# jnvance/DMRG.x

Measured on AMD Instinct MI355X. Metric: superblock MatMults/sec inside the ground-state eigensolve (Lanczos step = 1 MatMult + reorthogonalisation), higher is better.
Workload: dtype f64

## Files before the change

### dmrg.x_amd/csrc/ggemm.hip

```cpp
#include "ggemm.h"
#include <algorithm>
#include <cstdlib>
#include <map>
#include <mutex>
#include <utility>

namespace dmrgx {

typedef double d4 __attribute__((ext_vector_type(4)));

#ifdef DMRGX_TILE_TRACE
#define GG_TRACE_PARAM , unsigned long long* __restrict__ trace
#define GG_STAMP(I) { if (trace && threadIdx.x == 0) trace[(size_t)t * 8 + (I)] = __builtin_amdgcn_s_memrealtime(); }
#define GG_STAMP_ID() { if (trace && threadIdx.x == 0) { unsigned hw, xcc; asm volatile("s_getreg_b32 %0, hwreg(HW_REG_HW_ID)" : "=s"(hw)); asm volatile("s_getreg_b32 %0, hwreg(HW_REG_XCC_ID)" : "=s"(xcc)); trace[(size_t)t * 8 + 7] = ((unsigned long long)xcc << 32) | hw; } }
#define GG_TRACE_FWD , trace
#define GG_CLK0() unsigned long long clk0_ = __builtin_amdgcn_s_memtime();
#define GG_CLK1() { if (trace && threadIdx.x == 0) trace[(size_t)t * 8 + 6] = __builtin_amdgcn_s_memtime() - clk0_; }
#else
#define GG_TRACE_PARAM
#define GG_TRACE_FWD
#define GG_STAMP(I)
#define GG_STAMP_ID()
#define GG_CLK0()
#define GG_CLK1()
#endif
typedef const double __attribute__((address_space(1)))* gptr;
typedef double __attribute__((address_space(1)))* gwptr;
typedef const char __attribute__((address_space(1)))* gbptr;

typedef const GTile __attribute__((address_space(4)))* ktile_ptr;
typedef const GGroup __attribute__((address_space(4)))* kgroup_ptr;
typedef const GProd __attribute__((address_space(4)))* kprod_ptr;
__device__ __forceinline__ GTile kload(ktile_ptr p, int i) { GTile r; r.group = p[i].group; r.tm = p[i].tm; r.tn = p[i].tn; r.pad = p[i].pad; return r; }
__device__ __forceinline__ GGroup kload(kgroup_ptr p, int i)
{
    GGroup r;
    r.C = p[i].C; r.ldc = p[i].ldc; r.M = p[i].M; r.N = p[i].N; r.prod_begin = p[i].prod_begin; r.prod_end = p[i].prod_end;
    r.n_axpy = p[i].n_axpy; r.accumulate = p[i].accumulate;
    return r;
}
__device__ __forceinline__ GProd kload(kprod_ptr p, int i)
{
    GProd r;
    r.A = p[i].A; r.B = p[i].B; r.lda = p[i].lda; r.ldb = p[i].ldb; r.K = p[i].K; r.kind = p[i].kind; r.alpha = p[i].alpha;
    return r;
}


template <int TR, int TC, int WR, int WC, bool DEEP>
__device__ __forceinline__ void
ggemm_body(const GTile* __restrict__ tiles_, const GGroup* __restrict__ groups_, const GProd* __restrict__ prods_, int ntiles, int* __restrict__ ctr GG_TRACE_PARAM)
{
    const ktile_ptr tiles = (ktile_ptr)tiles_;
    const kgroup_ptr groups = (kgroup_ptr)groups_;
    const kprod_ptr prods = (kprod_ptr)prods_;
    constexpr int THREADS = 64 * WR * WC;
    constexpr int BM = 16 * TR * WR, BN = 16 * TC * WC, BK = GG_BK;
    constexpr int AS_LD = BK + 2;
    constexpr int BS_LD = BN + 16;
    constexpr int AROWS = THREADS / 16;
    constexpr int NA = BM / AROWS;
    constexpr int BROWS = THREADS / BN;
    constexpr int NB = BK / BROWS;
    constexpr bool RELAYOUT = (TR == 2 && TC == 2 && WR == 2 && WC == 2);
    extern __shared__ double gg_smem[];
    double (*As)[BM * AS_LD] = (double (*)[BM * AS_LD])gg_smem;
    double (*Bs)[BK * BS_LD] = (double (*)[BK * BS_LD])(gg_smem + 2 * BM * AS_LD);

    const int tid = threadIdx.x, wave = __builtin_amdgcn_readfirstlane(tid >> 6);
    int& sh_next = *(int*)(gg_smem + 2 * BM * AS_LD + 2 * BK * BS_LD);
    const int G = gridDim.x;
    const bool dyn = ntiles > G;
    const int xcd = blockIdx.x & 7, qbase = G >> 3;
    int t = blockIdx.x;
    GTile tl = kload(tiles, t);
    if (tl.group < 0) return;
    GGroup g = kload(groups, tl.group);
    const GTile tl_none = GTile{-1, 0, 0, 0};
#define GG_LANES()                                                                            \
    int tp_ = tid;                                                                            \
    asm volatile("" : "+v"(tp_));                                                             \
    const int a_r = tp_ >> 4, a_k = tp_ & 15, b_k = tp_ / BN, b_j = tp_ % BN;                 \
    (void)a_r; (void)a_k; (void)b_k; (void)b_j;
    unsigned st_a, st_b;
    {
        GG_LANES();
        st_a = (unsigned)(size_t)&As[0][a_r * AS_LD + a_k];
        st_b = (unsigned)(size_t)&Bs[0][b_k * BS_LD + b_j];
    }

    int lm0, ln0, lmrem, lnrem;
    double rc_a[NA], rc_b[NB];
    const double *cA = nullptr, *cB = nullptr;
    int clda = 0, cldb = 0, cK = 0;
    int lp = 0, lk = 0, lpend = 0;
    bool lmore = false;
    int kz[2] = {0, 0};
    int npre = 0;
    int vm_after = 0;

#define GG_LOADER_TILE(TL, GR)                                                                \
    {                                                                                         \
        lm0 = (TL).tm * GG_BM; ln0 = (TL).tn * GG_BN;                                         \
        lmrem = min(BM, (GR).M - lm0);                                                        \
        lnrem = min(BN, (GR).N - ln0);                                                        \
    }
#define GG_PRODUCT_SET(PR)                                                                    \
    {                                                                                         \
        cA = (PR).A; cB = (PR).B; clda = (PR).lda; cldb = (PR).ldb; cK = (PR).K;              \
        const int kc_ = min(cK, BK) - 1;                                                      \
        GG_LANES();                                                                           \
        const int bcol = min(b_j, lnrem - 1);                                                 \
        _Pragma("unroll") for (int s = 0; s < NA; ++s) aoff[s] = ((unsigned)min(a_r + AROWS * s, lmrem - 1) * (unsigned)clda + (unsigned)min(a_k, kc_)) * 8u; \
        _Pragma("unroll") for (int s = 0; s < NB; ++s) boff[s] = ((unsigned)min(b_k + BROWS * s, kc_) * (unsigned)cldb + (unsigned)bcol) * 8u; \
    }
#define GG_PRODUCT(P) { const GProd pr_ = kload(prods, P); GG_PRODUCT_SET(pr_); }
#define GG_RA_0_0 "v[96:97]"
#define GG_CA_0_0 "v96", "v97"
#define GG_RA_0_1 "v[98:99]"
#define GG_CA_0_1 "v98", "v99"
#define GG_RA_0_2 "v[100:101]"
#define GG_CA_0_2 "v100", "v101"
#define GG_RA_0_3 "v[102:103]"
#define GG_CA_0_3 "v102", "v103"
#define GG_RB_0_0 "v[104:105]"
#define GG_CB_0_0 "v104", "v105"
#define GG_RB_0_1 "v[106:107]"
#define GG_CB_0_1 "v106", "v107"
#define GG_RB_0_2 "v[108:109]"
#define GG_CB_0_2 "v108", "v109"
#define GG_RB_0_3 "v[110:111]"
#define GG_CB_0_3 "v110", "v111"
#define GG_RA_1_0 "v[112:113]"
#define GG_CA_1_0 "v112", "v113"
#define GG_RA_1_1 "v[114:115]"
#define GG_CA_1_1 "v114", "v115"
#define GG_RA_1_2 "v[116:117]"
#define GG_CA_1_2 "v116", "v117"
#define GG_RA_1_3 "v[118:119]"
#define GG_CA_1_3 "v118", "v119"
#define GG_RB_1_0 "v[120:121]"
#define GG_CB_1_0 "v120", "v121"
#define GG_RB_1_1 "v[122:123]"
#define GG_CB_1_1 "v122", "v123"
#define GG_RB_1_2 "v[124:125]"
#define GG_CB_1_2 "v124", "v125"
#define GG_RB_1_3 "v[126:127]"
#define GG_CB_1_3 "v126", "v127"
#define GG_ZT_0_0 "v_cndmask_b32_e64 v96, v96, 0, %0\n\tv_cndmask_b32_e64 v97, v97, 0, %0"
#define GG_ZT_0_1 "v_cndmask_b32_e64 v98, v98, 0, %0\n\tv_cndmask_b32_e64 v99, v99, 0, %0"
#define GG_ZT_0_2 "v_cndmask_b32_e64 v100, v100, 0, %0\n\tv_cndmask_b32_e64 v101, v101, 0, %0"
#define GG_ZT_0_3 "v_cndmask_b32_e64 v102, v102, 0, %0\n\tv_cndmask_b32_e64 v103, v103, 0, %0"
#define GG_ZT_1_0 "v_cndmask_b32_e64 v112, v112, 0, %0\n\tv_cndmask_b32_e64 v113, v113, 0, %0"
#define GG_ZT_1_1 "v_cndmask_b32_e64 v114, v114, 0, %0\n\tv_cndmask_b32_e64 v115, v115, 0, %0"
#define GG_ZT_1_2 "v_cndmask_b32_e64 v116, v116, 0, %0\n\tv_cndmask_b32_e64 v117, v117, 0, %0"
#define GG_ZT_1_3 "v_cndmask_b32_e64 v118, v118, 0, %0\n\tv_cndmask_b32_e64 v119, v119, 0, %0"
#define GG_LD1(OP, SET, S, OFFV, BASE, BREG) asm volatile("global_load_dwordx2 " GG_R##OP##_##SET##_##S ", %0, %1" : : "v"(OFFV), BREG(BASE) : "memory", GG_C##OP##_##SET##_##S)
#define GG_ST1(OP, SET, S, ADDR, OFFS) asm volatile("ds_write_b64 %0, " GG_R##OP##_##SET##_##S " offset:%1" : : "v"(ADDR), "i"(OFFS) : "memory")
#define GG_Z1(SET, S) asm volatile(GG_ZT_##SET##_##S : : "s"(zm_) : GG_CA_##SET##_##S)
#define GG_LOADER_NEXT()                                                                      \
    {                                                                                         \
        lk += BK;                                                                             \
        if (lk >= cK) { ++lp; lk = 0; if (lp < lpend) GG_PRODUCT(lp); }                       \
        lmore = lp < lpend;                                                                   \
    }
#define GG_LOADER_BASES()                                                                     \
        const int klast_ = cK - 1 - lk;                                                       \
        const int back_ = (klast_ < BK - 1 && cK >= BK) ? BK - 1 - klast_ : 0;                \
        const int kz_ = klast_ < BK - 1 ? (cK >= BK ? back_ : -(klast_ + 1)) : 0;             \
        gbptr A_ = (gbptr)(cA + (size_t)lm0 * clda + (lk - back_));                           \
        gbptr B_ = (gbptr)(cB + (size_t)(lk - back_) * cldb + ln0);
#define GG_GLOAD_D(SET)                                                                       \
    {                                                                                         \
        static_assert(!DEEP || (NA == 4 && NB == 4), "staging register table");               \
        GG_LOADER_BASES();                                                                    \
        kz[SET] = kz_;                                                                        \
        GG_LD1(A, SET, 0, aoff[0], A_, "{s[96:97]}"); GG_LD1(A, SET, 1, aoff[1 % NA], A_, "{s[96:97]}");   \
        GG_LD1(A, SET, 2, aoff[2 % NA], A_, "{s[96:97]}"); GG_LD1(A, SET, 3, aoff[3 % NA], A_, "{s[96:97]}");   \
        GG_LD1(B, SET, 0, boff[0], B_, "{s[98:99]}"); GG_LD1(B, SET, 1, boff[1 % NB], B_, "{s[98:99]}");   \
        GG_LD1(B, SET, 2, boff[2 % NB], B_, "{s[98:99]}"); GG_LD1(B, SET, 3, boff[3 % NB], B_, "{s[98:99]}");   \
        GG_LOADER_NEXT();                                                                     \
    }
#define GG_VMWAIT(N) asm volatile("s_waitcnt vmcnt(%0)" : : "n"(N) : "memory")
#define GG_LSTORE_D(BUF, SET)                                                                 \
    {                                                                                         \
        if (kz[SET] != 0) {                                                                   \
            GG_LANES();                                                                       \
            const unsigned long long zm_ = __builtin_amdgcn_ballot_w64(kz[SET] > 0 ? a_k < kz[SET] : a_k >= -kz[SET]);   \
            GG_Z1(SET, 0); GG_Z1(SET, 1); GG_Z1(SET, 2); GG_Z1(SET, 3);                       \
        }                                                                                     \
        GG_ST1(A, SET, 0, st_a, 8 * ((BUF) * BM * AS_LD + AROWS * 0 * AS_LD)); GG_ST1(A, SET, 1, st_a, 8 * ((BUF) * BM * AS_LD + AROWS * 1 * AS_LD)); \
        GG_ST1(A, SET, 2, st_a, 8 * ((BUF) * BM * AS_LD + AROWS * 2 * AS_LD)); GG_ST1(A, SET, 3, st_a, 8 * ((BUF) * BM * AS_LD + AROWS * 3 * AS_LD)); \
        GG_ST1(B, SET, 0, st_b, 8 * ((BUF) * BK * BS_LD + BROWS * 0 * BS_LD)); GG_ST1(B, SET, 1, st_b, 8 * ((BUF) * BK * BS_LD + BROWS * 1 * BS_LD)); \
        GG_ST1(B, SET, 2, st_b, 8 * ((BUF) * BK * BS_LD + BROWS * 2 * BS_LD)); GG_ST1(B, SET, 3, st_b, 8 * ((BUF) * BK * BS_LD + BROWS * 3 * BS_LD)); \
    }
#define GG_GLOAD_C()                                                                          \
    {                                                                                         \
        GG_LOADER_BASES();                                                                    \
        kz[0] = kz_;                                                                          \
        _Pragma("unroll") for (int s = 0; s < NA; ++s) rc_a[s] = *(gptr)(A_ + aoff[s]);       \
        _Pragma("unroll") for (int s = 0; s < NB; ++s) rc_b[s] = *(gptr)(B_ + boff[s]);       \
        GG_LOADER_NEXT();                                                                     \
    }
#define GG_LSTORE_C(BUF)                                                                      \
    {                                                                                         \
        if (kz[0] != 0) {                                                                     \
            GG_LANES();                                                                       \
            const bool z_ = kz[0] > 0 ? a_k < kz[0] : a_k >= -kz[0];                          \
            _Pragma("unroll") for (int s = 0; s < NA; ++s) rc_a[s] = z_ ? 0.0 : rc_a[s];      \
        }                                                                                     \
        _Pragma("unroll") for (int s = 0; s < NA; ++s)                                        \
            asm volatile("ds_write_b64 %0, %1 offset:%2" : : "v"(st_a), "v"(rc_a[s]), "i"(8 * ((BUF) * BM * AS_LD + AROWS * s * AS_LD)) : "memory"); \
        _Pragma("unroll") for (int s = 0; s < NB; ++s)                                        \
            asm volatile("ds_write_b64 %0, %1 offset:%2" : : "v"(st_b), "v"(rc_b[s]), "i"(8 * ((BUF) * BK * BS_LD + BROWS * s * BS_LD)) : "memory"); \
    }

#define GG_FRAG(SET, BUF, KK)                                                                 \
    {                                                                                         \
        _Pragma("unroll") for (int mi = 0; mi < TR; ++mi)                                     \
            asm volatile("ds_read_b64 %0, %1 offset:%2" : "=v"(fa[SET][mi]) : "v"(lds_a), "i"(8 * ((BUF) * BM * AS_LD + 16 * AS_LD * mi + (KK))) : "memory"); \
        _Pragma("unroll") for (int ni = 0; ni < TC; ++ni)                                     \
            asm volatile("ds_read_b64 %0, %1 offset:%2" : "=v"(fb[SET][ni]) : "v"(lds_b), "i"(8 * ((BUF) * BK * BS_LD + (KK) * BS_LD + 16 * ni)) : "memory"); \
    }
#define GG_FRAG_WAIT(SET)                                                                     \
    {                                                                                         \
        asm volatile("s_waitcnt lgkmcnt(0)" ::: "memory");                                    \
        _Pragma("unroll") for (int mi = 0; mi < TR; ++mi) asm volatile("" : "+v"(fa[SET][mi])); \
        _Pragma("unroll") for (int ni = 0; ni < TC; ++ni) asm volatile("" : "+v"(fb[SET][ni])); \
    }
#define GG_MFMA(SET, GUARD, I0, I1)       \
    {                                                                                         \
        _Pragma("unroll") for (int q = (I0); q < (I1); ++q) {                                 \
            const int mi = q / TC, ni = q % TC;                                               \
            GUARD(acc[mi][ni], fa[SET][mi], fb[SET][ni], q);                                  \
        }                                                                                     \
        __builtin_amdgcn_sched_barrier(0);                                                    \
    }
#define GG_CLAIM()                                                                            \
    asm volatile("s_mov_b64 s[94:95], exec\n\ts_mov_b64 exec, 1\n\tglobal_atomic_add %0, %1, %2, %3 sc0\n\ts_mov_b64 exec, s[94:95]" \
                 : "+v"(claim) : "v"(0u), "v"(1u), "{s[92:93]}"(ctr + xcd) : "memory", "s94", "s95")
#define GG_STEP_D(BUF, OTH, GUARD)                                                            \
    {                                                                                         \
        constexpr int NM = TR * TC;                                                           \
        GG_FRAG_WAIT(0);                                                                      \
        GG_MFMA(0, GUARD, 0, 1);                                                              \
        const bool ld_ = lmore;                                                               \
        __builtin_amdgcn_sched_barrier(0);                                                    \
        GG_MFMA(0, GUARD, 1, 2);                                                              \
        if (ld_) {                                                                            \
            GG_GLOAD_D(BUF);                                                                  \
            if (dyn && !lmore && wave == 0) GG_CLAIM();    \
        }                                                                                     \
        __builtin_amdgcn_sched_barrier(0);                                                    \
        GG_MFMA(0, GUARD, 2, NM - 1);                                                         \
        GG_FRAG(1, BUF, 4);                                                                   \
        GG_MFMA(0, GUARD, NM - 1, NM);                                                        \
        GG_FRAG_WAIT(1);                                                                      \
        GG_MFMA(1, GUARD, 0, NM - 1);                                                         \
        GG_FRAG(0, BUF, 8);                                                                   \
        GG_MFMA(1, GUARD, NM - 1, NM);                                                        \
        GG_FRAG_WAIT(0);                                                                      \
        GG_MFMA(0, GUARD, 0, 1);                                                              \
        if (have1) {                                                                          \
            if (ld_ && lmore) { GG_VMWAIT(NA + NB); } else { GG_VMWAIT(0); }    \
            GG_LSTORE_D(OTH, OTH);                                                            \
        }                                                                                     \
        __builtin_amdgcn_sched_barrier(0);                                                    \
        GG_MFMA(0, GUARD, 1, NM - 1);                                                         \
        GG_FRAG(1, BUF, 12);                                                                  \
        GG_MFMA(0, GUARD, NM - 1, NM);                                                        \
        GG_FRAG_WAIT(1);                                                                      \
        __syncthreads();                                                                      \
        if (have1) GG_FRAG(0, OTH, 0);                                                        \
        __builtin_amdgcn_sched_barrier(0);                                                    \
        GG_MFMA(1, GUARD, 0, NM);                                                             \
        have = have1; have1 = ld_;                                                            \
    }
#define GG_STEP_C(BUF, OTH, GUARD)                                                            \
    {                                                                                         \
        constexpr int NM = TR * TC;                                                           \
        GG_FRAG_WAIT(0);                                                                      \
        GG_MFMA(0, GUARD, 0, 1);                                                              \
        const bool ld_ = lmore;                                                               \
        __builtin_amdgcn_sched_barrier(0);                                                    \
        GG_MFMA(0, GUARD, 1, 2);                                                              \
        if (ld_) {                                                                            \
            GG_GLOAD_C();                                                                     \
            if (dyn && !lmore && wave == 0) GG_CLAIM();                                       \
        }                                                                                     \
        __builtin_amdgcn_sched_barrier(0);                                                    \
        GG_MFMA(0, GUARD, 2, NM - 1);                                                         \
        GG_FRAG(1, BUF, 4);                                                                   \
        GG_MFMA(0, GUARD, NM - 1, NM);                                                        \
        GG_FRAG_WAIT(1);                                                                      \
        GG_MFMA(1, GUARD, 0, NM - 1);                                                         \
        GG_FRAG(0, BUF, 8);                                                                   \
        GG_MFMA(1, GUARD, NM - 1, NM);                                                        \
        GG_FRAG_WAIT(0);                                                                      \
        GG_MFMA(0, GUARD, 0, 1);                                                              \
        if (ld_) GG_LSTORE_C(OTH);                                                            \
        __builtin_amdgcn_sched_barrier(0);                                                    \
        GG_MFMA(0, GUARD, 1, NM - 1);                                                         \
        GG_FRAG(1, BUF, 12);                                                                  \
        GG_MFMA(0, GUARD, NM - 1, NM);                                                        \
        GG_FRAG_WAIT(1);                                                                      \
        __syncthreads();                                                                      \
        if (ld_) GG_FRAG(0, OTH, 0);                                                          \
        __builtin_amdgcn_sched_barrier(0);                                                    \
        GG_MFMA(1, GUARD, 0, NM);                                                             \
        have = ld_;                                                                           \
    }
#define GG_STREAM(GUARD)                                                                      \
    while (have) {                                                                            \
        if (DEEP) { GG_STEP_D(0, 1, GUARD); } else { GG_STEP_C(0, 1, GUARD); }                \
        if (!have) break;                                                                     \
        if (DEEP) { GG_STEP_D(1, 0, GUARD); } else { GG_STEP_C(1, 0, GUARD); }                \
    }

    for (;;) {
        GG_STAMP(0);
        unsigned aoff[NA], boff[NB];
        const int m0 = tl.tm * GG_BM, n0 = tl.tn * GG_BN;
        const int mrem = min(BM, g.M - m0), nrem = min(BN, g.N - n0);
        int wrow = (wave / WC) * 16 * TR, wcol = (wave % WC) * 16 * TC;
        int tr_eff, tc_eff;
        if (RELAYOUT && mrem <= 32) {
            wrow = 0; wcol = 16 * wave;
            tr_eff = (mrem + 15) >> 4; tc_eff = nrem > wcol ? 1 : 0;
        } else if (RELAYOUT && nrem <= 32) {
            wrow = 16 * wave; wcol = 0;
            tr_eff = mrem > wrow ? 1 : 0; tc_eff = (nrem + 15) >> 4;
        } else {
            tr_eff = min(TR, max(0, (mrem - wrow + 15) >> 4)); tc_eff = min(TC, max(0, (nrem - wcol + 15) >> 4));
        }
        unsigned lds_a, lds_b;
        {
            int tf = tid;
            asm volatile("" : "+v"(tf));
            const int l15 = tf & 15, l4 = (tf >> 4) & 3;
            lds_a = (unsigned)(size_t)&As[0][(wrow + l15) * AS_LD + l4];
            lds_b = (unsigned)(size_t)&Bs[0][l4 * BS_LD + wcol + l15];
        }
        double fa[2][TR], fb[2][TC];

        d4 acc[TR][TC];
#pragma unroll
        for (int mi = 0; mi < TR; ++mi)
#pragma unroll
            for (int ni = 0; ni < TC; ++ni) acc[mi][ni] = (d4){0.0, 0.0, 0.0, 0.0};

        const int pend = g.prod_end;
        const int p0 = tl.pad >= 0 ? tl.pad : pend;
        if (npre == 0 && p0 < pend) {
            GG_LOADER_TILE(tl, g);
            lp = p0; lk = 0; lpend = pend;
            GG_PRODUCT(lp);
            GG_STAMP(1);
            vm_after = 0;
            if (DEEP) { GG_GLOAD_D(0); npre = 1; if (lmore) { GG_GLOAD_D(1); npre = 2; vm_after = NA + NB; } }
            else { GG_GLOAD_C(); npre = 1; }
        } else if (lmore) {
            GG_PRODUCT(lp);
        } else {
#pragma unroll
            for (int s = 0; s < NA; ++s) aoff[s] = 0u;
#pragma unroll
            for (int s = 0; s < NB; ++s) boff[s] = 0u;
        }
        bool have = npre >= 1, have1 = npre >= 2;
        (void)have1;
        if (have) {
            if (DEEP) {
                if (vm_after == NA + NB) { GG_VMWAIT(NA + NB); }
                else if (vm_after == NA + NB + TR * TC * 4) { GG_VMWAIT(NA + NB + TR * TC * 4); }
                else if (vm_after == TR * TC * 4) { GG_VMWAIT(TR * TC * 4); }
                else { GG_VMWAIT(0); }
                GG_LSTORE_D(0, 0);
            } else GG_LSTORE_C(0);
        }
        npre = 0;
        unsigned claim = 0xffffffffu;
        if (dyn && have && !lmore && wave == 0) GG_CLAIM();
        __syncthreads();
        GG_STAMP(2);
        GG_CLK0();
        if (have) GG_FRAG(0, 0, 0);
        unsigned gmask = 0;
#pragma unroll
        for (int q = 0; q < TR * TC; ++q) gmask |= ((q / TC) < tr_eff && (q % TC) < tc_eff) ? (1u << q) : 0u;
gmask = __builtin_amdgcn_readfirstlane(gmask);
#define GG_ALL(ACC, FA, FB, Q) ACC = __builtin_amdgcn_mfma_f64_16x16x4f64(FA, FB, ACC, 0, 0, 0)
#define GG_BIT(ACC, FA, FB, Q)                                                                \
        asm volatile("s_bitcmp1_b32 %3, %4\n\ts_cbranch_scc0 1f\n\tv_mfma_f64_16x16x4_f64 %0, %1, %2, %0\n1:" : "+v"(ACC) : "v"(FA), "v"(FB), "s"(gmask), "n"(Q) : "scc")
        if (TR * TC > 6) { GG_STREAM(GG_ALL) }
        else { GG_STREAM(GG_BIT) }
        GG_STAMP(3);
        GG_CLK1();
#pragma unroll
        for (int s = 0; s < NA; ++s) asm volatile("" : "=v"(rc_a[s]));
#pragma unroll
        for (int s = 0; s < NB; ++s) asm volatile("" : "=v"(rc_b[s]));
        int t_n = ntiles;
        if (dyn) {
            asm volatile("s_waitcnt vmcnt(0)" : "+v"(claim) : : "memory");
            if (tid == 0) sh_next = claim != 0xffffffffu ? (int)claim : (int)atomicAdd(&ctr[xcd], 1);
            __syncthreads();
            t_n = xcd + 8 * (__builtin_amdgcn_readfirstlane(sh_next) + qbase);
        }
        const GTile tl_n = t_n < ntiles ? kload(tiles, t_n) : tl_none;
        const bool nx = tl_n.group >= 0;
        GGroup g_n = g;
        GProd pr_n = GProd{nullptr, nullptr, 0, 0, 0, 0, 0.0};
        if (nx) g_n = kload(groups, tl_n.group);
        if (nx && tl_n.pad >= 0) pr_n = kload(prods, tl_n.pad);

        int tq = tid;
        asm volatile("" : "+v"(tq));
        const int el15 = tq & 15, el4 = (tq >> 4) & 3;
        const int erow = wrow + el4, ecol = wcol + el15;
        int q = g.prod_begin;
        const int axpy_end = q + g.n_axpy;
        const bool full_tile = mrem == BM && nrem == BN;
        if (DEEP && full_tile && q < axpy_end) {
#define GG_SREG_0 "v[96:97]"
#define GG_SCLB_0 "v96", "v97"
#define GG_SREG_1 "v[98:99]"
#define GG_SCLB_1 "v98", "v99"
#define GG_SREG_2 "v[100:101]"
#define GG_SCLB_2 "v100", "v101"
#define GG_SREG_3 "v[102:103]"
#define GG_SCLB_3 "v102", "v103"
#define GG_SREG_4 "v[104:105]"
#define GG_SCLB_4 "v104", "v105"
#define GG_SREG_5 "v[106:107]"
#define GG_SCLB_5 "v106", "v107"
#define GG_SREG_6 "v[108:109]"
#define GG_SCLB_6 "v108", "v109"
#define GG_SREG_7 "v[110:111]"
#define GG_SCLB_7 "v110", "v111"
#define GG_SREG_8 "v[112:113]"
#define GG_SCLB_8 "v112", "v113"
#define GG_SREG_9 "v[114:115]"
#define GG_SCLB_9 "v114", "v115"
#define GG_SREG_10 "v[116:117]"
#define GG_SCLB_10 "v116", "v117"
#define GG_SREG_11 "v[118:119]"
#define GG_SCLB_11 "v118", "v119"
#define GG_SREG_12 "v[120:121]"
#define GG_SCLB_12 "v120", "v121"
#define GG_SREG_13 "v[122:123]"
#define GG_SCLB_13 "v122", "v123"
#define GG_SREG_14 "v[124:125]"
#define GG_SCLB_14 "v124", "v125"
#define GG_SREG_15 "v[126:127]"
#define GG_SCLB_15 "v126", "v127"
#define GG_SLD(U, OFFV, BASE, IMM) asm volatile("global_load_dwordx2 " GG_SREG_##U ", %0, %1 offset:" #IMM : : "v"(OFFV), "{s[96:97]}"(BASE) : "memory", GG_SCLB_##U)
#define GG_SFMA(U, EL, AL) { double t_ = EL; asm volatile("v_fma_f64 %0, %1, " GG_SREG_##U ", %0" : "+v"(t_) : "s"(AL)); EL = t_; }
#define GG_SLOAD0(PR)                                                                         \
            {                                                                                 \
                const unsigned lo_ = ((unsigned)erow * (unsigned)(PR).ldb + (unsigned)ecol) * 8u;   \
                { gbptr S_ = (gbptr)((PR).B + (size_t)(m0 + 0 + 4 * 0) * (PR).ldb + n0); GG_SLD(0, lo_, S_, 0); GG_SLD(1, lo_, S_, 128); } \
                { gbptr S_ = (gbptr)((PR).B + (size_t)(m0 + 0 + 4 * 1) * (PR).ldb + n0); GG_SLD(2, lo_, S_, 0); GG_SLD(3, lo_, S_, 128); } \
                { gbptr S_ = (gbptr)((PR).B + (size_t)(m0 + 0 + 4 * 2) * (PR).ldb + n0); GG_SLD(4, lo_, S_, 0); GG_SLD(5, lo_, S_, 128); } \
                { gbptr S_ = (gbptr)((PR).B + (size_t)(m0 + 0 + 4 * 3) * (PR).ldb + n0); GG_SLD(6, lo_, S_, 0); GG_SLD(7, lo_, S_, 128); } \
            }
#define GG_SLOAD1(PR)                                                                         \
            {                                                                                 \
                const unsigned lo_ = ((unsigned)erow * (unsigned)(PR).ldb + (unsigned)ecol) * 8u;   \
                { gbptr S_ = (gbptr)((PR).B + (size_t)(m0 + 16 + 4 * 0) * (PR).ldb + n0); GG_SLD(8, lo_, S_, 0); GG_SLD(9, lo_, S_, 128); } \
                { gbptr S_ = (gbptr)((PR).B + (size_t)(m0 + 16 + 4 * 1) * (PR).ldb + n0); GG_SLD(10, lo_, S_, 0); GG_SLD(11, lo_, S_, 128); } \
                { gbptr S_ = (gbptr)((PR).B + (size_t)(m0 + 16 + 4 * 2) * (PR).ldb + n0); GG_SLD(12, lo_, S_, 0); GG_SLD(13, lo_, S_, 128); } \
                { gbptr S_ = (gbptr)((PR).B + (size_t)(m0 + 16 + 4 * 3) * (PR).ldb + n0); GG_SLD(14, lo_, S_, 0); GG_SLD(15, lo_, S_, 128); } \
            }
#define GG_SFMA0(AL)                                                                          \
            {                                                                                 \
                GG_SFMA(0, acc[0][0][0], AL); \
// ... 234 lines not shown
```

### dmrg.x_amd/csrc/kron_plan.hip

```cpp
#include "ggemm.h"
#include <algorithm>
#include <functional>
#include <map>
#include <set>
#include <tuple>
#include <cstring>
#include <memory>
#include <new>

namespace dmrgx {

namespace {

struct NCell {
    int32_t q, r0, c0, nr, nc, kind;
    double scale;
    const double* data;
    int64_t ld;
    bool tr;
};

struct PCell {
    int32_t q, r0, c0, nr, nc, kind;
    double scale;
// ... 414 lines not shown
    std::vector<Group> G;
    std::vector<CopyTask> copies;
    int64_t arena_ops = 0;
    auto new_dense = [&](int32_t nr, int32_t nc) { int64_t o = arena_ops; arena_ops += (int64_t)nr * nc; return o; };

    auto build_side = [&](const std::vector<std::pair<double, const std::vector<NCell>*>>& contrib, bool transpose_out, std::vector<PCell>& dst) {
        std::map<std::tuple<int32_t, int32_t, int32_t, int32_t, int32_t, int32_t>, int32_t> index;
        std::map<int32_t, int32_t> rounds;
        for (auto& ct : contrib) {
            for (const NCell& c : *ct.second) {
                auto key = std::make_tuple(c.q, c.r0, c.c0, c.nr, c.nc, c.kind);
                auto it = index.find(key);
                int32_t di;
                if (it == index.end()) {
                    PCell pc;
                    pc.kind = c.kind; pc.scale = 0.0; pc.off = -1;
                    if (!transpose_out) { pc.q = c.q; pc.r0 = c.r0; pc.c0 = c.c0; pc.nr = c.nr; pc.nc = c.nc; }
                    else { pc.q = c.q; pc.r0 = c.c0; pc.c0 = c.r0; pc.nr = c.nc; pc.nc = c.nr; }
                    if (c.kind == DMRGX_CELL_DENSE) pc.off = new_dense(pc.nr, pc.nc);
                    dst.push_back(pc);
                    di = (int32_t)dst.size() - 1;
                    index.emplace(key, di);
                } else di = it->second;
                if (c.kind == DMRGX_CELL_IDENT) dst[di].scale += ct.first * c.scale;
                else {
                    CopyTask k;
                    k.dst_off = dst[di].off; k.src = c.data; k.lds = c.ld;
                    k.nr = dst[di].nr; k.nc = dst[di].nc; k.ldd = dst[di].nc;
                    k.tr = (c.tr != transpose_out) ? 1 : 0;
                    k.a = ct.first; k.round = rounds[di]++;
                    copies.push_back(k);
                }
            }
        }
    };

    {
        std::map<std::pair<int32_t, int32_t>, std::vector<int32_t>> by_key;
        for (int32_t t = 0; t < d->nterms; ++t) {
            const dmrgx_term& T = d->terms[t];
            if (T.a == 0.0) continue;
            if (coverR[T.right_op]) by_key[{1, T.right_op}].push_back(t);
            else if (coverL[T.left_op]) by_key[{0, T.left_op}].push_back(t);
            else DMRGX_FAIL(DMRGX_ERR_INTERNAL, "kron_plan_create: term %d is not covered", t);
        }
        for (auto& kv : by_key) {
            Group g;
            std::vector<std::pair<double, const std::vector<NCell>*>> cl, cr;
            if (kv.first.first == 1) {
                g.sB = d->right_ops[kv.first.second].shift; g.sA = -g.sB;
                cr.push_back({1.0, &Rops[kv.first.second]});
                for (int32_t t : kv.second) cl.push_back({d->terms[t].a, &Lops[d->terms[t].left_op]});
            } else {
                g.sA = d->left_ops[kv.first.second].shift; g.sB = -g.sA;
                cl.push_back({1.0, &Lops[kv.first.second]});
                for (int32_t t : kv.second) cr.push_back({d->terms[t].a, &Rops[d->terms[t].right_op]});
            }
            build_side(cl, false, g.left);
            build_side(cr, true, g.rightT);
            G.push_back(std::move(g));
        }
    }
    std::vector<PCell> PHL, PHRT;
    build_side({{1.0, &HL}}, false, PHL);
    build_side({{1.0, &HR}}, true, PHRT);

    int64_t arena_T = 0;
    std::vector<std::vector<int64_t>> Toff(G.size(), std::vector<int64_t>(nb, -1));
    std::vector<std::vector<int32_t>> Ksrc(G.size(), std::vector<int32_t>(nb, -1));
    for (size_t g = 0; g < G.size(); ++g)
        for (int32_t k = 0; k < nb; ++k) {
            auto it = kmap.find({d->block_il[k] + G[g].sA, d->block_ir[k] + G[g].sB});
            if (it == kmap.end()) continue;
            Ksrc[g][k] = it->second;
            Toff[g][k] = arena_ops + arena_T;
            arena_T += (int64_t)nLk(it->second) * panel_ld(k, me);
        }
    std::vector<int64_t> TRoff(nb, -1);
    if (!PHRT.empty())
        for (int32_t k = 0; k < nb; ++k) { TRoff[k] = arena_ops + arena_T; arena_T += (int64_t)nLk(k) * panel_ld(k, me); }

    Builder B;
    std::vector<ZeroRect> zero_rects;
    auto stage1 = [&](const std::vector<PCell>& cellsT, int32_t sB, int32_t k, int32_t ksrc, int64_t toff) {
        (void)sB;
        const int32_t ir = d->block_ir[k], cs = cbeg(k, me), ce = cend(k, me), w = ce - cs;
        if (w <= 0) return;
        const int32_t M = nLk(ksrc);
        std::set<int32_t> cuts = {cs, ce};
        auto clampc = [&](int32_t v) { return std::min(std::max(v, cs), ce); };
        for (const PCell& c : cellsT) {
            if (c.q != ir) continue;
            cuts.insert(clampc(c.c0)); cuts.insert(clampc(c.c0 + c.nc));
            if (c.kind == DMRGX_CELL_IDENT)
                for (int32_t p = 0; p < W; ++p) { const int32_t sc = cbeg(ksrc, p); if (sc > c.r0 && sc < c.r0 + c.nr) cuts.insert(clampc(c.c0 + (sc - c.r0))); }
        }
        std::vector<int32_t> cv(cuts.begin(), cuts.end());
        for (size_t s = 0; s + 1 < cv.size(); ++s) {
            const int32_t o0 = cv[s], o1 = cv[s + 1];
            if (o0 >= o1) continue;
            bool any = false;
            for (const PCell& c : cellsT) if (c.q == ir && c.c0 <= o0 && c.c0 + c.nc >= o1) { any = true; break; }
            if (!any) { zero_rects.push_back(ZeroRect{toff + (o0 - cs), w, M, o1 - o0, 0}); continue; }
            const int32_t g = B.open(BASE_ARENA, toff + (o0 - cs), w, M, o1 - o0, 0);
            for (const PCell& c : cellsT) {
                if (c.q != ir || c.c0 > o0 || c.c0 + c.nc < o1) continue;
                if (c.kind == DMRGX_CELL_DENSE) {
                    for (int32_t p = 0; p < W; ++p) {
                        const int32_t k0 = std::max(c.r0, cbeg(ksrc, p)), k1 = std::min(c.r0 + c.nr, cend(ksrc, p));
                        if (k0 >= k1) continue;
                        B.add_gemm(BASE_X, panel_off(ksrc, p) + (k0 - cbeg(ksrc, p)), panel_ld(ksrc, p),
                                   BASE_ARENA, c.off + (int64_t)(k0 - c.r0) * c.nc + (o0 - c.c0), c.nc, k1 - k0);
                    }
                } else {
                    const int32_t s0 = c.r0 + (o0 - c.c0);
                    int32_t p = 0;
                    for (int32_t pp = 0; pp < W; ++pp) if (cbeg(ksrc, pp) <= s0 && s0 < cend(ksrc, pp)) p = pp;
                    B.add_axpy(BASE_X, panel_off(ksrc, p) + (s0 - cbeg(ksrc, p)), panel_ld(ksrc, p), c.scale);
                }
            }
            B.close(g, 1);
        }
    };
    for (size_t g = 0; g < G.size(); ++g)
        for (int32_t k = 0; k < nb; ++k) if (Ksrc[g][k] >= 0) stage1(G[g].rightT, G[g].sB, k, Ksrc[g][k], Toff[g][k]);
    if (!PHRT.empty()) for (int32_t k = 0; k < nb; ++k) stage1(PHRT, 0, k, k, TRoff[k]);
    const int32_t n_groups_stage1 = (int32_t)B.groups.size();

    for (int32_t k = 0; k < nb; ++k) {
        const int32_t il = d->block_il[k], w = panel_ld(k, me), nl = nLk(k);
        if (w <= 0) continue;
        std::set<int32_t> cuts = {0, nl};
        for (size_t g = 0; g < G.size(); ++g) if (Ksrc[g][k] >= 0) for (const PCell& c : G[g].left) if (c.q == il) { cuts.insert(c.r0); cuts.insert(c.r0 + c.nr); }
        for (const PCell& c : PHL) if (c.q == il) { cuts.insert(c.r0); cuts.insert(c.r0 + c.nr); }
        std::vector<int32_t> cv(cuts.begin(), cuts.end());
        for (size_t s = 0; s + 1 < cv.size(); ++s) {
            const int32_t ra = cv[s], rb = cv[s + 1];
            const int32_t grp = B.open(BASE_Y, seg_off[me][k] + (int64_t)ra * w, w, rb - ra, w, 0);
            for (size_t g = 0; g < G.size(); ++g) {
                if (Ksrc[g][k] < 0) continue;
                for (const PCell& c : G[g].left) {
                    if (c.q != il || c.r0 > ra || c.r0 + c.nr < rb) continue;
                    if (c.kind == DMRGX_CELL_DENSE)
                        B.add_gemm(BASE_ARENA, c.off + (int64_t)(ra - c.r0) * c.nc, c.nc, BASE_ARENA, Toff[g][k] + (int64_t)c.c0 * w, w, c.nc);
                    else
                        B.add_axpy(BASE_ARENA, Toff[g][k] + (int64_t)(c.c0 + (ra - c.r0)) * w, w, c.scale);
                }
            }
            for (const PCell& c : PHL) {
                if (c.q != il || c.r0 > ra || c.r0 + c.nr < rb) continue;
                if (c.kind == DMRGX_CELL_DENSE)
                    B.add_gemm(BASE_ARENA, c.off + (int64_t)(ra - c.r0) * c.nc, c.nc, BASE_X, panel_off(k, me) + (int64_t)c.c0 * w, w, c.nc);
                else
                    B.add_axpy(BASE_X, panel_off(k, me) + (int64_t)(c.c0 + (ra - c.r0)) * w, w, c.scale);
            }
            if (TRoff[k] >= 0) B.add_axpy(BASE_ARENA, TRoff[k] + (int64_t)ra * w, w, 1.0);
            B.close(grp, 2);
        }
    }

    const int64_t slab_base = arena_ops + arena_T;
    B.finalize_stage2(slab_base);
    const int64_t arena_slabs = B.slab_elems;
    ggemm_schedule(B.tiles1, B.groups);
    ggemm_schedule(B.tiles2, B.groups);
    ggemm_schedule(B.tiles1b, B.groups, 2);
    ggemm_schedule(B.tiles2b, B.groups, 2);
    if (const char* dump = getenv("DMRGX_PLAN_DUMP")) {
        if (FILE* f = fopen(dump, "w")) {
            auto put = [&](const char* name, const std::vector<GTile>& tl) {
                for (size_t i = 0; i < tl.size(); ++i) {
                    const GTile& t = tl[i];
                    if (t.group < 0) { fprintf(f, "%s %zu -1 0 0 0 0 0 0\n", name, i); continue; }
                    const RelGroup& G2 = B.groups[t.group];
                    fprintf(f, "%s %zu %d %d %d %d %d %d %d\n", name, i, t.group, t.tm, t.tn, G2.M, G2.N, B.ksteps(t.group), G2.prod_end - G2.prod_begin);
                }
            };
            put("s1", B.tiles1); put("s2", B.tiles2); put("s1b", B.tiles1b); put("s2b", B.tiles2b);
            for (size_t i = 0; i < zero_rects.size(); ++i) {
                const ZeroRect& z = zero_rects[i];
                fprintf(f, "zr %zu %lld %d %d %d\n", i, (long long)z.off, z.ld, z.nr, z.nc);
            }
            for (size_t i = 0; i < B.red_tasks.size(); ++i) {
                const RedTask& r = B.red_tasks[i];
                fprintf(f, "red %zu %lld %lld %d %d %d %d\n", i, (long long)r.dst_off, (long long)r.slab_off, r.ldc, r.M, r.N, r.nslab);
            }
            fclose(f);
        }
    }

    dmrgx_kron_plan* P = new (std::nothrow) dmrgx_kron_plan();
    if (!P) DMRGX_FAIL(DMRGX_ERR_MEM, "out of host memory");
    std::unique_ptr<dmrgx_kron_plan> guard(P);
    P->world = W; P->rank = me;
    DMRGX_CHK(P->arena.alloc_f64((size_t)std::max<int64_t>(arena_ops + arena_T + arena_slabs, 1), st));
    P->n_red_tiles = (int32_t)B.red_tiles.size();
    {
        int32_t max_round = -1;
        for (auto& c : copies) max_round = std::max(max_round, c.round);
        DevBuf d_tab;
        PackedUpload pk;
        const size_t o_tasks = pk.add(copies);
        const size_t o_zero = pk.add(zero_rects);
        std::vector<std::pair<size_t, size_t>> lists;
        for (int32_t r = 0; r <= max_round; ++r) {
            std::vector<CopyTile> ct;
            for (size_t i = 0; i < copies.size(); ++i) if (copies[i].round == r)
                for (int32_t ti = 0; ti < (copies[i].nr + 31) / 32; ++ti)
                    for (int32_t tj = 0; tj < (copies[i].nc + 31) / 32; ++tj) ct.push_back(CopyTile{(int32_t)i, ti, tj, 0});
            if (ct.empty()) continue;
            lists.push_back({pk.add(ct), ct.size()});
        }
        DMRGX_CHK(pk.upload(d_tab, st));
        if (!zero_rects.empty()) {
            int64_t big = 1;
            for (const ZeroRect& r : zero_rects) big = std::max(big, (int64_t)r.nr * r.nc);
            if (zero_rects.size() >= ((size_t)1 << 23)) DMRGX_FAIL(DMRGX_ERR_ARG, "kron_plan: %zu zero rectangles exceed the launch grid", zero_rects.size());
            hipLaunchKernelGGL(zero_rects_kernel, dim3((unsigned)zero_rects.size(), (unsigned)std::min<int64_t>((big + 2047) / 2048, 512)), dim3(256), 0, st,
                               (const ZeroRect*)packed_at<ZeroRect>(d_tab, o_zero), P->arena.as<double>());
            DMRGX_HIP(hipGetLastError());
        }
        for (const auto& l : lists) {
            hipLaunchKernelGGL(cell_copy_kernel, dim3((unsigned)l.second), dim3(256), 0, st, (const CopyTile*)packed_at<CopyTile>(d_tab, l.first), (const CopyTask*)packed_at<CopyTask>(d_tab, o_tasks), P->arena.as<double>());
            DMRGX_HIP(hipGetLastError());
        }
    }
    P->nprods = (int32_t)B.prods.size(); P->ngroups = (int32_t)B.groups.size();
    P->ntiles1 = (int32_t)B.tiles1.size(); P->ntiles2 = (int32_t)B.tiles2.size();
    P->ntiles1b = (int32_t)B.tiles1b.size(); P->ntiles2b = (int32_t)B.tiles2b.size();
    {
        std::vector<LayoutSeg> segs;
        for (int32_t k = 0; k < nb; ++k) for (int32_t w = 0; w < W; ++w) {
            if (panel_ld(k, w) <= 0) continue;
            segs.push_back(LayoutSeg{ref_off[k] + cbeg(k, w), panel_off(k, w), nLk(k), panel_ld(k, w), nRk(k), panel_ld(k, w)});
        }
        P->nlayout = (int32_t)segs.size();
        PackedUpload pk;
        const size_t o0 = pk.add(B.prods), o1 = pk.add(B.groups), o2 = pk.add(B.tiles1), o3 = pk.add(B.tiles2), o4 = pk.add(B.tiles1b), o5 = pk.add(B.tiles2b),
                     o8 = pk.add(B.red_tasks), o9 = pk.add(B.red_tiles), o10 = pk.add(segs);
        DMRGX_CHK(pk.upload(P->d_tables, st));
// ... 198 lines not shown
```

Baseline: 366.5.

## Skip structurally zero tiles in two-stage Kronecker GEMM plan and mask zero K-chunks

Stage-1 groups are split into row-tile ranges, and tiles whose rows are never read by any stage-2 left cell get no GEMM work. Stage-2 groups are split into column-tile ranges, and products whose intermediate tile was never written (structurally zero) are dropped. Their flops are still counted in flops_alg. In the kernel, the K-padding information for each buffer selects per-kstep MFMA masks, so MFMAs on fully zero-padded 4-wide K slices are skipped. This cuts wasted MFMA and memory work, but produces more, smaller groups and more plan-time bookkeeping.

```diff
diff --git a/dmrg.x_amd/csrc/ggemm.hip b/dmrg.x_amd/csrc/ggemm.hip
--- a/dmrg.x_amd/csrc/ggemm.hip
+++ b/dmrg.x_amd/csrc/ggemm.hip
@@ -96,6 +96,7 @@
     int lp = 0, lk = 0, lpend = 0;
     bool lmore = false;
     int kz[2] = {0, 0};
+    int kzb[2] = {0, 0};
     int npre = 0;
     int vm_after = 0;
 
@@ -184,6 +185,7 @@
 #define GG_VMWAIT(N) asm volatile("s_waitcnt vmcnt(%0)" : : "n"(N) : "memory")
 #define GG_LSTORE_D(BUF, SET)                                                                 \
     {                                                                                         \
+        kzb[BUF] = kz[SET];                                                                   \
         if (kz[SET] != 0) {                                                                   \
             GG_LANES();                                                                       \
             const unsigned long long zm_ = __builtin_amdgcn_ballot_w64(kz[SET] > 0 ? a_k < kz[SET] : a_k >= -kz[SET]);   \
@@ -228,86 +230,95 @@
         _Pragma("unroll") for (int mi = 0; mi < TR; ++mi) asm volatile("" : "+v"(fa[SET][mi])); \
         _Pragma("unroll") for (int ni = 0; ni < TC; ++ni) asm volatile("" : "+v"(fb[SET][ni])); \
     }
-#define GG_MFMA(SET, GUARD, I0, I1)       \
+#define GG_MFMA(SET, GUARD, MASK, I0, I1)       \
     {                                                                                         \
         _Pragma("unroll") for (int q = (I0); q < (I1); ++q) {                                 \
             const int mi = q / TC, ni = q % TC;                                               \
-            GUARD(acc[mi][ni], fa[SET][mi], fb[SET][ni], q);                                  \
+            GUARD(acc[mi][ni], fa[SET][mi], fb[SET][ni], q, MASK);                            \
         }                                                                                     \
         __builtin_amdgcn_sched_barrier(0);                                                    \
     }
 #define GG_CLAIM()                                                                            \
     asm volatile("s_mov_b64 s[94:95], exec\n\ts_mov_b64 exec, 1\n\tglobal_atomic_add %0, %1, %2, %3 sc0\n\ts_mov_b64 exec, s[94:95]" \
                  : "+v"(claim) : "v"(0u), "v"(1u), "{s[92:93]}"(ctr + xcd) : "memory", "s94", "s95")
+#define GG_KMASKS(KZ)                                                                         \
+        const int kzs_ = (KZ);                                                                \
+        const int klo_ = max(kzs_, 0), khi_ = kzs_ < 0 ? -kzs_ : BK;                          \
+        const unsigned km0_ = 4 > klo_ ? gmask : 0u;                                          \
+        const unsigned km1_ = (8 > klo_ && 4 < khi_) ? gmask : 0u;                            \
+        const unsigned km2_ = (12 > klo_ && 8 < khi_) ? gmask : 0u;                           \
+        const unsigned km3_ = 12 < khi_ ? gmask : 0u;                                         \
+        (void)km0_; (void)km1_; (void)km2_; (void)km3_;
 #define GG_STEP_D(BUF, OTH, GUARD)                                                            \
     {                                                                                         \
         constexpr int NM = TR * TC;                                                           \
+        GG_KMASKS(kzb[BUF]);                                                                  \
         GG_FRAG_WAIT(0);                                                                      \
-        GG_MFMA(0, GUARD, 0, 1);                                                              \
+        GG_MFMA(0, GUARD, km0_, 0, 1);                                                              \
         const bool ld_ = lmore;                                                               \
         __builtin_amdgcn_sched_barrier(0);                                                    \
-        GG_MFMA(0, GUARD, 1, 2);                                                              \
+        GG_MFMA(0, GUARD, km0_, 1, 2);                                                              \
         if (ld_) {                                                                            \
             GG_GLOAD_D(BUF);                                                                  \
             if (dyn && !lmore && wave == 0) GG_CLAIM();    \
         }                                                                                     \
         __builtin_amdgcn_sched_barrier(0);                                                    \
-        GG_MFMA(0, GUARD, 2, NM - 1);                                                         \
+        GG_MFMA(0, GUARD, km0_, 2, NM - 1);                                                         \
         GG_FRAG(1, BUF, 4);                                                                   \
-        GG_MFMA(0, GUARD, NM - 1, NM);                                                        \
+        GG_MFMA(0, GUARD, km0_, NM - 1, NM);                                                        \
         GG_FRAG_WAIT(1);                                                                      \
-        GG_MFMA(1, GUARD, 0, NM - 1);                                                         \
+        GG_MFMA(1, GUARD, km1_, 0, NM - 1);                                                         \
         GG_FRAG(0, BUF, 8);                                                                   \
-        GG_MFMA(1, GUARD, NM - 1, NM);                                                        \
+        GG_MFMA(1, GUARD, km1_, NM - 1, NM);                                                        \
         GG_FRAG_WAIT(0);                                                                      \
-        GG_MFMA(0, GUARD, 0, 1);                                                              \
+        GG_MFMA(0, GUARD, km2_, 0, 1);                                                              \
         if (have1) {                                                                          \
             if (ld_ && lmore) { GG_VMWAIT(NA + NB); } else { GG_VMWAIT(0); }    \
             GG_LSTORE_D(OTH, OTH);                                                            \
         }                                                                                     \
         __builtin_amdgcn_sched_barrier(0);                                                    \
-        GG_MFMA(0, GUARD, 1, NM - 1);                                                         \
+        GG_MFMA(0, GUARD, km2_, 1, NM - 1);                                                         \
         GG_FRAG(1, BUF, 12);                                                                  \
-        GG_MFMA(0, GUARD, NM - 1, NM);                                                        \
+        GG_MFMA(0, GUARD, km2_, NM - 1, NM);                                                        \
         GG_FRAG_WAIT(1);                                                                      \
         __syncthreads();                                                                      \
         if (have1) GG_FRAG(0, OTH, 0);                                                        \
         __builtin_amdgcn_sched_barrier(0);                                                    \
-        GG_MFMA(1, GUARD, 0, NM);                                                             \
+        GG_MFMA(1, GUARD, km3_, 0, NM);                                                             \
         have = have1; have1 = ld_;                                                            \
     }
 #define GG_STEP_C(BUF, OTH, GUARD)                                                            \
     {                                                                                         \
         constexpr int NM = TR * TC;                                                           \
         GG_FRAG_WAIT(0);                                                                      \
-        GG_MFMA(0, GUARD, 0, 1);                                                              \
+        GG_MFMA(0, GUARD, gmask, 0, 1);                                                              \
         const bool ld_ = lmore;                                                               \
         __builtin_amdgcn_sched_barrier(0);                                                    \
-        GG_MFMA(0, GUARD, 1, 2);                                                              \
+        GG_MFMA(0, GUARD, gmask, 1, 2);                                                              \
         if (ld_) {                                                                            \
             GG_GLOAD_C();                                                                     \
             if (dyn && !lmore && wave == 0) GG_CLAIM();                                       \
         }                                                                                     \
         __builtin_amdgcn_sched_barrier(0);                                                    \
-        GG_MFMA(0, GUARD, 2, NM - 1);                                                         \
+        GG_MFMA(0, GUARD, gmask, 2, NM - 1);                                                         \
         GG_FRAG(1, BUF, 4);                                                                   \
-        GG_MFMA(0, GUARD, NM - 1, NM);                                                        \
+        GG_MFMA(0, GUARD, gmask, NM - 1, NM);                                                        \
         GG_FRAG_WAIT(1);                                                                      \
-        GG_MFMA(1, GUARD, 0, NM - 1);                                                         \
+        GG_MFMA(1, GUARD, gmask, 0, NM - 1);                                                         \
         GG_FRAG(0, BUF, 8);                                                                   \
-        GG_MFMA(1, GUARD, NM - 1, NM);                                                        \
+        GG_MFMA(1, GUARD, gmask, NM - 1, NM);                                                        \
         GG_FRAG_WAIT(0);                                                                      \
-        GG_MFMA(0, GUARD, 0, 1);                                                              \
+        GG_MFMA(0, GUARD, gmask, 0, 1);                                                              \
         if (ld_) GG_LSTORE_C(OTH);                                                            \
         __builtin_amdgcn_sched_barrier(0);                                                    \
-        GG_MFMA(0, GUARD, 1, NM - 1);                                                         \
+        GG_MFMA(0, GUARD, gmask, 1, NM - 1);                                                         \
         GG_FRAG(1, BUF, 12);                                                                  \
-        GG_MFMA(0, GUARD, NM - 1, NM);                                                        \
+        GG_MFMA(0, GUARD, gmask, NM - 1, NM);                                                        \
         GG_FRAG_WAIT(1);                                                                      \
         __syncthreads();                                                                      \
         if (ld_) GG_FRAG(0, OTH, 0);                                                          \
         __builtin_amdgcn_sched_barrier(0);                                                    \
-        GG_MFMA(1, GUARD, 0, NM);                                                             \
+        GG_MFMA(1, GUARD, gmask, 0, NM);                                                             \
         have = ld_;                                                                           \
     }
 #define GG_STREAM(GUARD)                                                                      \
@@ -389,9 +400,9 @@
 #pragma unroll
         for (int q = 0; q < TR * TC; ++q) gmask |= ((q / TC) < tr_eff && (q % TC) < tc_eff) ? (1u << q) : 0u;
 gmask = __builtin_amdgcn_readfirstlane(gmask);
-#define GG_ALL(ACC, FA, FB, Q) ACC = __builtin_amdgcn_mfma_f64_16x16x4f64(FA, FB, ACC, 0, 0, 0)
-#define GG_BIT(ACC, FA, FB, Q)                                                                \
-        asm volatile("s_bitcmp1_b32 %3, %4\n\ts_cbranch_scc0 1f\n\tv_mfma_f64_16x16x4_f64 %0, %1, %2, %0\n1:" : "+v"(ACC) : "v"(FA), "v"(FB), "s"(gmask), "n"(Q) : "scc")
+#define GG_ALL(ACC, FA, FB, Q, MASK) ACC = __builtin_amdgcn_mfma_f64_16x16x4f64(FA, FB, ACC, 0, 0, 0)
+#define GG_BIT(ACC, FA, FB, Q, MASK)                                                          \
+        asm volatile("s_bitcmp1_b32 %3, %4\n\ts_cbranch_scc0 1f\n\tv_mfma_f64_16x16x4_f64 %0, %1, %2, %0\n1:" : "+v"(ACC) : "v"(FA), "v"(FB), "s"(MASK), "n"(Q) : "scc")
         if (TR * TC > 6) { GG_STREAM(GG_ALL) }
         else { GG_STREAM(GG_BIT) }
         GG_STAMP(3);
diff --git a/dmrg.x_amd/csrc/kron_plan.hip b/dmrg.x_amd/csrc/kron_plan.hip
--- a/dmrg.x_amd/csrc/kron_plan.hip
+++ b/dmrg.x_amd/csrc/kron_plan.hip
@@ -520,11 +520,11 @@
 
     Builder B;
     std::vector<ZeroRect> zero_rects;
-    auto stage1 = [&](const std::vector<PCell>& cellsT, int32_t sB, int32_t k, int32_t ksrc, int64_t toff) {
+    auto stage1 = [&](const std::vector<PCell>& cellsT, int32_t sB, int32_t k, int32_t ksrc, int64_t toff, const std::vector<char>* rread) {
         (void)sB;
         const int32_t ir = d->block_ir[k], cs = cbeg(k, me), ce = cend(k, me), w = ce - cs;
         if (w <= 0) return;
-        const int32_t M = nLk(ksrc);
+        const int32_t M = nLk(ksrc), mt = (M + GG_BM - 1) / GG_BM;
         std::set<int32_t> cuts = {cs, ce};
         auto clampc = [&](int32_t v) { return std::min(std::max(v, cs), ce); };
         for (const PCell& c : cellsT) {
@@ -540,60 +540,105 @@
             bool any = false;
             for (const PCell& c : cellsT) if (c.q == ir && c.c0 <= o0 && c.c0 + c.nc >= o1) { any = true; break; }
             if (!any) { zero_rects.push_back(ZeroRect{toff + (o0 - cs), w, M, o1 - o0, 0}); continue; }
-            const int32_t g = B.open(BASE_ARENA, toff + (o0 - cs), w, M, o1 - o0, 0);
+            for (int32_t t0 = 0, t1; t0 < mt; t0 = t1) {
+                const bool rd = !rread || (*rread)[t0];
+                for (t1 = t0 + 1; t1 < mt && (!rread || ((*rread)[t1] != 0) == rd); ++t1) {}
+                const int32_t m0 = t0 * GG_BM, m1 = std::min(M, t1 * GG_BM);
+                const double mn = (double)(m1 - m0) * (o1 - o0);
+                const int32_t g = B.open(BASE_ARENA, toff + (int64_t)m0 * w + (o0 - cs), w, m1 - m0, o1 - o0, 0);
+                for (const PCell& c : cellsT) {
+                    if (c.q != ir || c.c0 > o0 || c.c0 + c.nc < o1) continue;
+                    if (c.kind == DMRGX_CELL_DENSE) {
+                        for (int32_t p = 0; p < W; ++p) {
+                            const int32_t k0 = std::max(c.r0, cbeg(ksrc, p)), k1 = std::min(c.r0 + c.nr, cend(ksrc, p));
+                            if (k0 >= k1) continue;
+                            if (!rd) { B.flops_alg += 2.0 * mn * (k1 - k0); continue; }
+                            B.add_gemm(BASE_X, panel_off(ksrc, p) + (int64_t)m0 * panel_ld(ksrc, p) + (k0 - cbeg(ksrc, p)), panel_ld(ksrc, p),
+                                       BASE_ARENA, c.off + (int64_t)(k0 - c.r0) * c.nc + (o0 - c.c0), c.nc, k1 - k0);
+                        }
+                    } else {
+                        if (!rd) { B.flops_alg += 2.0 * mn; continue; }
+                        const int32_t s0 = c.r0 + (o0 - c.c0);
+                        int32_t p = 0;
+                        for (int32_t pp = 0; pp < W; ++pp) if (cbeg(ksrc, pp) <= s0 && s0 < cend(ksrc, pp)) p = pp;
+                        B.add_axpy(BASE_X, panel_off(ksrc, p) + (int64_t)m0 * panel_ld(ksrc, p) + (s0 - cbeg(ksrc, p)), panel_ld(ksrc, p), c.scale);
+                    }
+                }
+                B.close(g, 1);
+            }
+        }
+    };
+    std::vector<char> rread;
+    for (size_t g = 0; g < G.size(); ++g)
+        for (int32_t k = 0; k < nb; ++k) {
+            if (Ksrc[g][k] < 0) continue;
+            rread.assign((nLk(Ksrc[g][k]) + GG_BM - 1) / GG_BM, 0);
+            for (const PCell& c : G[g].left)
+                if (c.q == d->block_il[k]) for (int32_t t = c.c0 / GG_BM; t <= (c.c0 + c.nc - 1) / GG_BM; ++t) rread[t] = 1;
+            stage1(G[g].rightT, G[g].sB, k, Ksrc[g][k], Toff[g][k], &rread);
+        }
+    if (!PHRT.empty()) for (int32_t k = 0; k < nb; ++k) stage1(PHRT, 0, k, k, TRoff[k], nullptr);
+    const int32_t n_groups_stage1 = (int32_t)B.groups.size();
+
+    for (int32_t k = 0; k < nb; ++k) {
+        const int32_t il = d->block_il[k], ir = d->block_ir[k], w = panel_ld(k, me), nl = nLk(k), cs = cbeg(k, me), ce = cend(k, me);
+        if (w <= 0) continue;
+        const int32_t nt = (w + GG_BN - 1) / GG_BN, sR = (int32_t)G.size();
+        std::vector<std::vector<char>> reach(G.size() + 1, std::vector<char>(nt, 0));
+        auto mark = [&](const std::vector<PCell>& cellsT, std::vector<char>& r) {
             for (const PCell& c : cellsT) {
-                if (c.q != ir || c.c0 > o0 || c.c0 + c.nc < o1) continue;
-                if (c.kind == DMRGX_CELL_DENSE) {
-                    for (int32_t p = 0; p < W; ++p) {
-                        const int32_t k0 = std::max(c.r0, cbeg(ksrc, p)), k1 = std::min(c.r0 + c.nr, cend(ksrc, p));
-                        if (k0 >= k1) continue;
-                        B.add_gemm(BASE_X, panel_off(ksrc, p) + (k0 - cbeg(ksrc, p)), panel_ld(ksrc, p),
-                                   BASE_ARENA, c.off + (int64_t)(k0 - c.r0) * c.nc + (o0 - c.c0), c.nc, k1 - k0);
-                    }
-                } else {
-                    const int32_t s0 = c.r0 + (o0 - c.c0);
-                    int32_t p = 0;
-                    for (int32_t pp = 0; pp < W; ++pp) if (cbeg(ksrc, pp) <= s0 && s0 < cend(ksrc, pp)) p = pp;
-                    B.add_axpy(BASE_X, panel_off(ksrc, p) + (s0 - cbeg(ksrc, p)), panel_ld(ksrc, p), c.scale);
-                }
-            }
-            B.close(g, 1);
-        }
-    };
-    for (size_t g = 0; g < G.size(); ++g)
-        for (int32_t k = 0; k < nb; ++k) if (Ksrc[g][k] >= 0) stage1(G[g].rightT, G[g].sB, k, Ksrc[g][k], Toff[g][k]);
-    if (!PHRT.empty()) for (int32_t k = 0; k < nb; ++k) stage1(PHRT, 0, k, k, TRoff[k]);
-    const int32_t n_groups_stage1 = (int32_t)B.groups.size();
-
-    for (int32_t k = 0; k < nb; ++k) {
-        const int32_t il = d->block_il[k], w = panel_ld(k, me), nl = nLk(k);
-        if (w <= 0) continue;
+                if (c.q != ir) continue;
+                const int32_t o0 = std::min(std::max(c.c0, cs), ce) - cs, o1 = std::min(std::max(c.c0 + c.nc, cs), ce) - cs;
+                for (int32_t t = o0 / GG_BN; o0 < o1 && t <= (o1 - 1) / GG_BN; ++t) r[t] = 1;
+            }
+        };
+        for (size_t g = 0; g < G.size(); ++g) if (Ksrc[g][k] >= 0) mark(G[g].rightT, reach[g]);
+        if (TRoff[k] >= 0) mark(PHRT, reach[sR]);
         std::set<int32_t> cuts = {0, nl};
         for (size_t g = 0; g < G.size(); ++g) if (Ksrc[g][k] >= 0) for (const PCell& c : G[g].left) if (c.q == il) { cuts.insert(c.r0); cuts.insert(c.r0 + c.nr); }
         for (const PCell& c : PHL) if (c.q == il) { cuts.insert(c.r0); cuts.insert(c.r0 + c.nr); }
         std::vector<int32_t> cv(cuts.begin(), cuts.end());
         for (size_t s = 0; s + 1 < cv.size(); ++s) {
             const int32_t ra = cv[s], rb = cv[s + 1];
-            const int32_t grp = B.open(BASE_Y, seg_off[me][k] + (int64_t)ra * w, w, rb - ra, w, 0);
+            std::vector<int32_t> used;
             for (size_t g = 0; g < G.size(); ++g) {
                 if (Ksrc[g][k] < 0) continue;
-                for (const PCell& c : G[g].left) {
+                for (const PCell& c : G[g].left) if (c.q == il && c.r0 <= ra && c.r0 + c.nr >= rb) { used.push_back((int32_t)g); break; }
+            }
+            if (TRoff[k] >= 0) used.push_back(sR);
+            for (int32_t t0 = 0, t1; t0 < nt; t0 = t1) {
+                for (t1 = t0 + 1; t1 < nt; ++t1) {
+                    bool same = true;
+                    for (int32_t u : used) if (reach[u][t1] != reach[u][t0]) { same = false; break; }
+                    if (!same) break;
+                }
+                const int32_t c0 = t0 * GG_BN, c1 = std::min(w, t1 * GG_BN);
+                const double mn = (double)(rb - ra) * (c1 - c0);
+                const int32_t grp = B.open(BASE_Y, seg_off[me][k] + (int64_t)ra * w + c0, w, rb - ra, c1 - c0, 0);
+                for (size_t g = 0; g < G.size(); ++g) {
+                    if (Ksrc[g][k] < 0) continue;
+                    for (const PCell& c : G[g].left) {
+                        if (c.q != il || c.r0 > ra || c.r0 + c.nr < rb) continue;
+                        if (!reach[g][t0]) { B.flops_alg += c.kind == DMRGX_CELL_DENSE ? 2.0 * mn * c.nc : 2.0 * mn; continue; }
+                        if (c.kind == DMRGX_CELL_DENSE)
+                            B.add_gemm(BASE_ARENA, c.off + (int64_t)(ra - c.r0) * c.nc, c.nc, BASE_ARENA, Toff[g][k] + (int64_t)c.c0 * w + c0, w, c.nc);
+                        else
+                            B.add_axpy(BASE_ARENA, Toff[g][k] + (int64_t)(c.c0 + (ra - c.r0)) * w + c0, w, c.scale);
+                    }
+                }
+                for (const PCell& c : PHL) {
                     if (c.q != il || c.r0 > ra || c.r0 + c.nr < rb) continue;
                     if (c.kind == DMRGX_CELL_DENSE)
-                        B.add_gemm(BASE_ARENA, c.off + (int64_t)(ra - c.r0) * c.nc, c.nc, BASE_ARENA, Toff[g][k] + (int64_t)c.c0 * w, w, c.nc);
+                        B.add_gemm(BASE_ARENA, c.off + (int64_t)(ra - c.r0) * c.nc, c.nc, BASE_X, panel_off(k, me) + (int64_t)c.c0 * w + c0, w, c.nc);
                     else
-                        B.add_axpy(BASE_ARENA, Toff[g][k] + (int64_t)(c.c0 + (ra - c.r0)) * w, w, c.scale);
+                        B.add_axpy(BASE_X, panel_off(k, me) + (int64_t)(c.c0 + (ra - c.r0)) * w + c0, w, c.scale);
                 }
-            }
-            for (const PCell& c : PHL) {
-                if (c.q != il || c.r0 > ra || c.r0 + c.nr < rb) continue;
-                if (c.kind == DMRGX_CELL_DENSE)
-                    B.add_gemm(BASE_ARENA, c.off + (int64_t)(ra - c.r0) * c.nc, c.nc, BASE_X, panel_off(k, me) + (int64_t)c.c0 * w, w, c.nc);
-                else
-                    B.add_axpy(BASE_X, panel_off(k, me) + (int64_t)(c.c0 + (ra - c.r0)) * w, w, c.scale);
-            }
-            if (TRoff[k] >= 0) B.add_axpy(BASE_ARENA, TRoff[k] + (int64_t)ra * w, w, 1.0);
-            B.close(grp, 2);
+                if (TRoff[k] >= 0) {
+                    if (reach[sR][t0]) B.add_axpy(BASE_ARENA, TRoff[k] + (int64_t)ra * w + c0, w, 1.0);
+                    else B.flops_alg += 2.0 * mn;
+                }
+                B.close(grp, 2);
+            }
         }
     }
 
```

After: 369.7 (median of 6 runs). About the same (+0.9%).
